# EarthyScience/EasyHybrid.jl

Measured on NVIDIA B200. Metric: training samples/sec (fwd+bwd+Adam), higher is better.
Workload: dtype f32

## Files before the change

### easyhybrid.jl_b200/csrc/eh_chunk.cuh

```cuda
#pragma once
#include "eh_pm.cuh"

namespace eh {

constexpr int MAXP = 12;
constexpr int EH_MAX_WORLD = 8;
constexpr int BS_C = 0, BS_N = MAXT, BS_SS = 2 * MAXT, BS_BN = 3 * MAXT, BS_AFF = 3 * MAXT + 2 * MAXP, BS_STRIDE = BS_AFF + 4 * MAXT;

enum : int { OPT_ADAM = 0, OPT_ADAMW = 1, OPT_RMSPROP = 2, OPT_DESCENT = 3 };
enum : int { UPD_FULL = 0, UPD_REDUCE_ONLY = 1, UPD_FROM_VECTOR = 2 };

struct OptState {
    float b1t, b2t;
    long long t;
    long long skipped;
};

struct PSlot {
    int role;
    int idx;
    float lo;
    float span;
    float fixedv;
};

template <int P_, int NH_, int H_, int NOUT_, int ACT_, bool SCALE_, class PM_, int SPL_ = 1>
struct StepCfg {
    static constexpr int P = P_, NH = NH_, H = H_, NOUT = NOUT_, ACT = ACT_;
    static constexpr bool SCALE = SCALE_;
    static constexpr int SPL = SPL_;
    static constexpr int CHUNKS = 32 * SPL_;
    static constexpr int RS = CHUNKS + 4;
    using PM = PM_;
    static constexpr int F = PM::NF, T = PM::NT, NPS = PM::NPS;
    static constexpr int LR = (NOUT_ * (H_ + 1) + PM_::NT + PM_::NPS <= 32) ? 1 : 0;
    static constexpr ShapeDims D{P_, NH_, H_, NOUT_, LR};
    static constexpr int NLAST = NOUT_ * (H_ + 1);
    static constexpr int R4 = rup4(P_ + PM::NF + PM::NT);
    static constexpr int NB = D.nblocks();
    static constexpr int NBI = (NB + 31) / 32;
    static constexpr int NBP = NB | 1;
    static constexpr int SCR_PAD = (NBP - NB) * 16;
    static constexpr int SCR = D.npart() + SCR_PAD;
    static constexpr int GS = 4 * RS + 4;
    static constexpr int AUXOFF = D.ngroups() * GS;
    static constexpr int STAGE_FLOATS = AUXOFF + (ACT_ == ACT_SWISH ? NH_ * H_ * RS : 0);
    static constexpr int NW = D.nweights();
    static constexpr int NPART = D.npart();
    static_assert(P_ <= MAXP && H_ % 4 == 0 && NOUT_ <= 4 && (SPL_ == 1 || SPL_ == 2), "shape limits");
};

constexpr int SS_SLOT = 0, SS_PMS = 16, SS_C = 48, SS_NV = 52, SS_BN = 56, SS_NV2 = 80, SS_SGD = 96, SS_AFF = 104, SS_FLOATS = 128;

template <int RS>
__device__ __forceinline__ constexpr int goff(int g0, int k) { return (g0 + (k >> 2)) * (4 * RS + 4) + (k & 3) * RS; }

__device__ __forceinline__ float comp(const float2* v, int k) { return (k & 1) ? v[k >> 1].y : v[k >> 1].x; }

template <int S>
__device__ __forceinline__ void stage_put(float* row, int lane, const float (&v)[S])
{
    if (S == 2) *reinterpret_cast<float2*>(row + 2 * lane) = f2(v[0], v[S - 1]);
    else row[lane] = v[0];
}
template <int S>
__device__ __forceinline__ void stage_get(const float* row, int lane, float (&v)[S])
{
    if (S == 2) {
        float2 t = *reinterpret_cast<const float2*>(row + 2 * lane);
        v[0] = t.x;
        v[S - 1] = t.y;
    } else {
        v[0] = row[lane];
    }
}

template <class C>
__device__ __forceinline__ float2 unit_act_fwd2(int l, int j2, float2 z, float2& aux)
// ... 42 lines not shown
        for (int k = 0; k < P; k++) {
            const float4* w4 = reinterpret_cast<const float4*>(sW + D.off_w1f() + k * H);
#pragma unroll
            for (int j = 0; j < HP; j += 2) {
                float4 w = w4[j >> 1];
                hp[j] = fma2s(f2(w.x, w.y), x[k], hp[j]);
                hp[j + 1] = fma2s(f2(w.z, w.w), x[k], hp[j + 1]);
            }
        }
    }
#pragma unroll
    for (int l = 1; l <= NH; l++) {
#pragma unroll
        for (int j = 0; j < HP; j++) {
            float2 aux = f2s(0.f);
            const float2 z = hp[j];
            hp[j] = unit_act_fwd2<C>(l, 2 * j, hp[j], aux);
            if (C::PM::DYNAMIC && pass) {
                const unsigned m = pass[l - 1] >> (2 * j);
                if (m & 1u) hp[j].x = z.x;
                if (m & 2u) hp[j].y = z.y;
            }
            if (STAGE && l + 1 <= D.nlt()) {
                stage[goff<RS>(D.gA(l + 1), 2 * j) + lane] = hp[j].x;
                stage[goff<RS>(D.gA(l + 1), 2 * j + 1) + lane] = hp[j].y;
            }
            if (STAGE) {
                if (C::ACT == ACT_SWISH) {
                    stage[C::AUXOFF + ((l - 1) * H + 2 * j) * RS + lane] = aux.x;
                    stage[C::AUXOFF + ((l - 1) * H + 2 * j + 1) * RS + lane] = aux.y;
                }
            }
        }
        if (l < NH) {
            float2 z[HP];
            const float4* b4 = reinterpret_cast<const float4*>(sW + D.off_b(l + 1));
#pragma unroll
            for (int j = 0; j < HP; j += 2) {
                float4 b = b4[j >> 1];
                z[j] = f2(b.x, b.y);
                z[j + 1] = f2(b.z, b.w);
            }
#pragma unroll
            for (int k = 0; k < H; k++) {
                const float4* w4 = reinterpret_cast<const float4*>(sW + D.off_wf(l + 1) + k * H);
                const float ak = comp(hp, k);
#pragma unroll
                for (int j = 0; j < HP; j += 2) {
// ... 47 lines not shown
    }
}

template <class C>
__device__ __forceinline__ void load_weights_and_scalars(const float* pblock, int nflat, const int* wsrc,
                                                         const float* bscal, int use_bn, float* sW, float* sS)
{
    for (int i = threadIdx.x; i < C::NW; i += blockDim.x) {
        int s = wsrc[i];
        sW[i] = s >= 0 ? __ldcg(pblock + s) : (s == -2 ? 1.f : 0.f);
    }
    if (threadIdx.x < MAXPS) sS[SS_SLOT + threadIdx.x] = __ldcg(pblock + nflat + threadIdx.x);
    if (threadIdx.x < MAXPS * PMS_PER_SLOT) sS[SS_PMS + threadIdx.x] = __ldcg(pblock + nflat + MAXPS + threadIdx.x);
    if (threadIdx.x < MAXT) sS[SS_C + threadIdx.x] = bscal ? bscal[BS_C + threadIdx.x] : 0.f;
    if (threadIdx.x < 2 * C::P)
        sS[SS_BN + threadIdx.x] = use_bn ? bscal[BS_BN + threadIdx.x] : ((threadIdx.x & 1) ? 1.f : 0.f);
    if (threadIdx.x < 3 * MAXT) sS[SS_AFF + threadIdx.x] = bscal ? bscal[BS_AFF + threadIdx.x] : 0.f;
}

template <class C>
__device__ __forceinline__ void init_stage_rows(float* stage, int lane)
{
    constexpr ShapeDims D = C::D;
    constexpr int RS = C::RS, S = C::SPL;
    float one[S], zero[S];
#pragma unroll
    for (int i = 0; i < S; i++) { one[i] = 1.f; zero[i] = 0.f; }
#pragma unroll
    for (int l = 1; l <= D.nlt(); l++) {
        const int din = D.din(l), ka = D.ka(l), gA = D.gA(l);
#pragma unroll
        for (int k = din; k < ka; k++) stage_put<S>(stage + goff<RS>(gA, k), lane, (k == din) ? one : zero);
    }
    if (!C::LR) {
#pragma unroll
        for (int o = C::NOUT; o < rup4(C::NOUT); o++) stage_put<S>(stage + goff<RS>(D.gD(C::NH + 1), o), lane, zero);
    }
}

template <class C>
__device__ __forceinline__ void tile_rows(int lane, int* rowD, int* rowA)
{
    constexpr ShapeDims D = C::D;
#pragma unroll
    for (int i = 0; i < C::NBI; i++) {
        int b = lane + 32 * i;
        rowD[i] = 0;
        rowA[i] = 0;
#pragma unroll
        for (int l = 1; l <= D.nlt(); l++) {
            const int b0 = D.blk0(l), nk = D.nk(l), nb = D.nj(l) * nk;
            if (b >= b0 && b < b0 + nb) {
                int jb = (b - b0) / nk, kb = (b - b0) % nk;
                rowD[i] = (D.gD(l) + jb) * C::GS;
                rowA[i] = (D.gA(l) + kb) * C::GS;
            }
        }
    }
}
// ... 35 lines not shown
        }
    }
};

template <class C>
__device__ __forceinline__ void chunk_sample_phase(const float (*rec)[C::R4], const bool* valid, const float* sW,
                                                   const float* sS, float* stage, int lane, const PSlot* slot,
                                                   const int* loss_kind, const PmCtx& cx, ChunkStats& st, LastAcc<C>& la)
{
    constexpr ShapeDims D = C::D;
    constexpr int P = C::P, NH = C::NH, H = C::H, NOUT = C::NOUT, T = C::T, F = C::F, NPS = C::NPS, HP = C::H / 2;
    constexpr int RS = C::RS, S = C::SPL;
    using PM = typename C::PM;

    float x[S][P];
#pragma unroll
    for (int k = 0; k < P; k++) {
        float v[S];
#pragma unroll
        for (int s = 0; s < S; s++) {
            x[s][k] = (rec[s][k] - sS[SS_BN + 2 * k]) * sS[SS_BN + 2 * k + 1];
            v[s] = x[s][k];
        }
        stage_put<S>(stage + goff<RS>(D.gA(1), k), lane, v);
    }

    float2 hp[S][HP];
    {
        const float4* b4 = reinterpret_cast<const float4*>(sW + D.off_b1());
#pragma unroll
        for (int j = 0; j < HP; j += 2) {
            float4 b = b4[j >> 1];
#pragma unroll
            for (int s = 0; s < S; s++) { hp[s][j] = f2(b.x, b.y); hp[s][j + 1] = f2(b.z, b.w); }
        }
#pragma unroll
        for (int k = 0; k < P; k++) {
            const float4* w4 = reinterpret_cast<const float4*>(sW + D.off_w1f() + k * H);
#pragma unroll
            for (int j = 0; j < HP; j += 2) {
                float4 w = w4[j >> 1];
#pragma unroll
                for (int s = 0; s < S; s++) {
                    hp[s][j] = fma2s(f2(w.x, w.y), x[s][k], hp[s][j]);
                    hp[s][j + 1] = fma2s(f2(w.z, w.w), x[s][k], hp[s][j + 1]);
                }
            }
        }
    }
#pragma unroll
    for (int l = 1; l <= NH; l++) {
#pragma unroll
        for (int j = 0; j < HP; j++) {
            float lo[S], hi[S], axl[S], axh[S];
#pragma unroll
            for (int s = 0; s < S; s++) {
                float2 aux = f2s(0.f);
                const float2 z = hp[s][j];
                hp[s][j] = unit_act_fwd2<C>(l, 2 * j, hp[s][j], aux);
                if (C::PM::DYNAMIC) {
                    const unsigned m = cx.pass[l - 1] >> (2 * j);
                    if (m & 1u) hp[s][j].x = z.x;
                    if (m & 2u) hp[s][j].y = z.y;
                }
                lo[s] = hp[s][j].x; hi[s] = hp[s][j].y; axl[s] = aux.x; axh[s] = aux.y;
            }
            if (l + 1 <= D.nlt()) {
                stage_put<S>(stage + goff<RS>(D.gA(l + 1), 2 * j), lane, lo);
                stage_put<S>(stage + goff<RS>(D.gA(l + 1), 2 * j + 1), lane, hi);
            }
            if (C::ACT == ACT_SWISH) {
                stage_put<S>(stage + C::AUXOFF + ((l - 1) * H + 2 * j) * RS, lane, axl);
                stage_put<S>(stage + C::AUXOFF + ((l - 1) * H + 2 * j + 1) * RS, lane, axh);
            }
        }
        if (l < NH) {
            float2 z[S][HP];
            const float4* b4 = reinterpret_cast<const float4*>(sW + D.off_b(l + 1));
#pragma unroll
            for (int j = 0; j < HP; j += 2) {
                float4 b = b4[j >> 1];
#pragma unroll
                for (int s = 0; s < S; s++) { z[s][j] = f2(b.x, b.y); z[s][j + 1] = f2(b.z, b.w); }
            }
#pragma unroll
            for (int k = 0; k < H; k++) {
                const float4* w4 = reinterpret_cast<const float4*>(sW + D.off_wf(l + 1) + k * H);
                float ak[S];
#pragma unroll
                for (int s = 0; s < S; s++) ak[s] = comp(hp[s], k);
#pragma unroll
                for (int j = 0; j < HP; j += 2) {
// ... 73 lines not shown
#pragma unroll
                for (int o = 0; o < NOUT; o++)
                    if (sl.idx == o) dz[s][o] += g;
            } else if (sl.role == ROLE_GLOBAL) {
                st.gphi[q] += gp[q];
            }
        }
    }
    if (C::LR) {
#pragma unroll
        for (int o = 0; o < NOUT; o++)
#pragma unroll
            for (int s = 0; s < S; s++) {
                la.b[o] += dz[s][o];
#pragma unroll
                for (int k = 0; k < HP; k++) la.w[o][k] = fma2s(hp[s][k], dz[s][o], la.w[o][k]);
            }
    } else {
#pragma unroll
        for (int o = 0; o < NOUT; o++) {
            float v[S];
#pragma unroll
            for (int s = 0; s < S; s++) v[s] = dz[s][o];
            stage_put<S>(stage + goff<RS>(D.gD(NH + 1), o), lane, v);
        }
    }

    float2 d[S][HP];
#pragma unroll
    for (int s = 0; s < S; s++)
#pragma unroll
        for (int k = 0; k < HP; k++) d[s][k] = f2s(0.f);
#pragma unroll
    for (int o = 0; o < NOUT; o++) {
        const float4* w4 = reinterpret_cast<const float4*>(sW + D.off_wo() + o * H);
#pragma unroll
        for (int k = 0; k < HP; k += 2) {
            float4 w = w4[k >> 1];
#pragma unroll
            for (int s = 0; s < S; s++) {
                d[s][k] = fma2s(f2(w.x, w.y), dz[s][o], d[s][k]);
                d[s][k + 1] = fma2s(f2(w.z, w.w), dz[s][o], d[s][k + 1]);
            }
        }
    }
#pragma unroll
    for (int l = NH; l >= 1; l--) {
#pragma unroll
        for (int k = 0; k < HP; k++) {
            float alo[S], ahi[S], xlo[S], xhi[S], dlo[S], dhi[S];
            if (l < NH) {
                stage_get<S>(stage + goff<RS>(D.gA(l + 1), 2 * k), lane, alo);
                stage_get<S>(stage + goff<RS>(D.gA(l + 1), 2 * k + 1), lane, ahi);
            }
            if (C::ACT == ACT_SWISH) {
                stage_get<S>(stage + C::AUXOFF + ((l - 1) * H + 2 * k) * RS, lane, xlo);
                stage_get<S>(stage + C::AUXOFF + ((l - 1) * H + 2 * k + 1) * RS, lane, xhi);
            }
#pragma unroll
            for (int s = 0; s < S; s++) {
                float2 al = (l < NH) ? f2(alo[s], ahi[s]) : hp[s][k];
                float2 aux = (C::ACT == ACT_SWISH) ? f2(xlo[s], xhi[s]) : f2s(0.f);
                float2 ga = unit_act_bwd2<C>(l, 2 * k, al, aux);
                if (C::PM::DYNAMIC) {
                    const unsigned m = cx.pass[l - 1] >> (2 * k);
                    if (m & 1u) ga.x = 1.f;
                    if (m & 2u) ga.y = 1.f;
                }
                d[s][k] = mul2(d[s][k], ga);
                dlo[s] = d[s][k].x;
                dhi[s] = d[s][k].y;
            }
            stage_put<S>(stage + goff<RS>(D.gD(l), 2 * k), lane, dlo);
            stage_put<S>(stage + goff<RS>(D.gD(l), 2 * k + 1), lane, dhi);
        }
        if (l > 1) {
            float2 dn[S][HP];
#pragma unroll
            for (int s = 0; s < S; s++)
#pragma unroll
                for (int k = 0; k < HP; k++) dn[s][k] = f2s(0.f);
#pragma unroll
            for (int j = 0; j < H; j++) {
                const float4* w4 = reinterpret_cast<const float4*>(sW + D.off_wb(l) + j * H);
                float dj[S];
#pragma unroll
                for (int s = 0; s < S; s++) dj[s] = comp(d[s], j);
#pragma unroll
                for (int k = 0; k < HP; k += 2) {
                    float4 w = w4[k >> 1];
#pragma unroll
                    for (int s = 0; s < S; s++) {
                        dn[s][k] = fma2s(f2(w.x, w.y), dj[s], dn[s][k]);
                        dn[s][k + 1] = fma2s(f2(w.z, w.w), dj[s], dn[s][k + 1]);
                    }
                }
            }
// ... 24 lines not shown
                float4 dv[4], av[4];
#pragma unroll
                for (int j = 0; j < 4; j++) dv[j] = *reinterpret_cast<const float4*>(pd + j * RS + c);
#pragma unroll
                for (int k = 0; k < 4; k++) av[k] = *reinterpret_cast<const float4*>(pa + k * RS + c);
#pragma unroll
                for (int j = 0; j < 4; j++)
#pragma unroll
                    for (int k = 0; k < 4; k++) {
                        acc[j * 4 + k] = fma2(f2(dv[j].x, dv[j].y), f2(av[k].x, av[k].y), acc[j * 4 + k]);
                        acc[j * 4 + k] = fma2(f2(dv[j].z, dv[j].w), f2(av[k].z, av[k].w), acc[j * 4 + k]);
                    }
            }
#pragma unroll
            for (int e = 0; e < 16; e++) wacc[e * C::NBP + b] = acc[e].x + acc[e].y;
        }
    }
}

template <class C>
__device__ __forceinline__ void chunk_dw_phase_mma(const float* stage, int lane, float* wacc, bool first)
{
    constexpr ShapeDims D = C::D;
    constexpr int RS = C::RS;
    static_assert(C::H % 16 == 0 && C::LR == 1 && C::SPL == 1, "tensor-pipe dW: hidden width multiple of 16, output layer in registers");
    constexpr int MT = C::H / 16;
    const int g = lane >> 2, t = lane & 3;
#pragma unroll
    for (int l = 1; l <= D.nlt(); l++) {
        const int ka = D.ka(l), nk = D.nk(l), b0 = D.blk0(l);
        const int NT = (ka + 7) / 8;
        float acc[MT][6][4];
#pragma unroll
        for (int mt = 0; mt < MT; mt++)
#pragma unroll
            for (int nt = 0; nt < 6; nt++)
#pragma unroll
                for (int q = 0; q < 4; q++) acc[mt][nt][q] = 0.f;
#pragma unroll
        for (int ks = 0; ks < C::CHUNKS / 8; ks++) {
            const int k0 = 8 * ks + t;
            unsigned bh[6][2], bl[6][2];
#pragma unroll
            for (int nt = 0; nt < 6; nt++) {
                if (nt < NT) {
                    const float* pb = stage + goff<RS>(D.gA(l), 8 * nt + g) + k0;
                    split_tf32(pb[0], bh[nt][0], bl[nt][0]);
                    split_tf32(pb[4], bh[nt][1], bl[nt][1]);
                }
            }
#pragma unroll
            for (int mt = 0; mt < MT; mt++) {
                const float* pa0 = stage + goff<RS>(D.gD(l), 16 * mt + g) + k0;
                const float* pa1 = stage + goff<RS>(D.gD(l), 16 * mt + g + 8) + k0;
                unsigned ah[4], al[4];
                split_tf32(pa0[0], ah[0], al[0]);
                split_tf32(pa1[0], ah[1], al[1]);
                split_tf32(pa0[4], ah[2], al[2]);
                split_tf32(pa1[4], ah[3], al[3]);
#pragma unroll
                for (int nt = 0; nt < 6; nt++)
                    if (nt < NT) mma_3xtf32(acc[mt][nt], ah, al, bh[nt], bl[nt]);
            }
        }
#pragma unroll
        for (int mt = 0; mt < MT; mt++)
#pragma unroll
            for (int nt = 0; nt < 6; nt++) {
                if (nt < NT) {
#pragma unroll
                    for (int q = 0; q < 4; q++) {
                        const int j = 16 * mt + g + ((q >> 1) ? 8 : 0), k = 8 * nt + 2 * t + (q & 1);
                        if (k < ka) {
                            const int cell = ((j & 3) * 4 + (k & 3)) * C::NBP + b0 + (j >> 2) * nk + (k >> 2);
                            wacc[cell] = first ? acc[mt][nt][q] : wacc[cell] + acc[mt][nt][q];
                        }
                    }
// ... 85 lines not shown
```

### easyhybrid.jl_b200/csrc/eh_engine_ffma.cuh

```cuda
#pragma once
#include "eh_chunk.cuh"

namespace eh {

template <class C>
struct EngFfma {
    using Cfg = C;
    static constexpr int ENGINE = C::SPL == 2 ? 2 : 0;
    static constexpr int STAGE_FLOATS = C::STAGE_FLOATS + rup4(C::SCR);
    static constexpr int NPART = C::NPART;
    static constexpr int OFF_STATS = C::D.npart_dw();
    static constexpr int CHUNK = C::CHUNKS;
    static constexpr int MAX_WARPS = C::SPL == 2 ? 10 : 16;
#ifdef EH_DW_FFMA
    static constexpr bool DW_MMA = false;
#else
    static constexpr bool DW_MMA = C::LR == 1 && C::H % 16 == 0 && C::SPL == 1 && C::D.ka(C::D.nlt()) <= 48;
#endif

    struct State {
        int nacc;
        ChunkStats st;
        LastAcc<C> la;
        int rowD[C::NBI], rowA[C::NBI];
        float4 r[C::SPL][C::R4 / 4];
        bool valid[C::SPL];
    };

    __device__ __forceinline__ static void init_warp(State& s, float* stage, int lane)
    {
        init_stage_rows<C>(stage, lane);
        tile_rows<C>(lane, s.rowD, s.rowA);
    }
    __device__ __forceinline__ static void after_reduce(State&, float*, int) {}
    __device__ __forceinline__ static void step_begin(State& s, const float* sW, int lane)
    {
        s.nacc = 0;
#pragma unroll
        for (int t = 0; t < MAXT; t++) s.st.loss[t] = 0.f;
#pragma unroll
        for (int t = 0; t < MAXPS; t++) s.st.gphi[t] = 0.f;
// ... 50 lines not shown
```

### easyhybrid.jl_b200/csrc/eh_engine_tc.cuh

```cuda
#pragma once
#include <cstdint>
#include "eh_engine_ffma.cuh"

namespace eh {

namespace tc {
constexpr int WPS = 256;
constexpr int ENG_WF_H = 0, ENG_WF_L = 4 * WPS, ENG_WB_H = 8 * WPS, ENG_WB_L = 12 * WPS, ENG_BAR = 16 * WPS, ENG_TMEM = ENG_BAR + 8 * 8,
              ENG_BYTES = ENG_TMEM + 16;
constexpr int COL_AH = 0, COL_AL = 16, COL_Z = 32, COLS_PER_GROUP = 64;

__device__ __forceinline__ uint32_t saddr(const void* p) { return (uint32_t)__cvta_generic_to_shared(p); }
__device__ __forceinline__ uint64_t desc(uint32_t sa, uint32_t lbo, uint32_t sbo)
{
    return (uint64_t)((sa & 0x3FFFF) >> 4) | ((uint64_t)((lbo >> 4) & 0x3FFF) << 16) | ((uint64_t)((sbo >> 4) & 0x3FFF) << 32) | ((uint64_t)1 << 46);
}
__host__ __device__ constexpr uint32_t idesc(int m, int n)
{
    return (1u << 4) | (2u << 7) | (2u << 10) | ((uint32_t)(n >> 3) << 17) | ((uint32_t)(m >> 4) << 24);
}
__device__ __forceinline__ void mma_ts(uint32_t d, uint32_t a, uint64_t b, uint32_t id, uint32_t acc)
{
    asm volatile(
        "{\n\t.reg .pred p;\n\tsetp.ne.b32 p, %4, 0;\n\t"
// ... 170 lines not shown
    __device__ __forceinline__ static void step_begin(State& s, const float*, int)
    {
        s.nacc = 0;
#pragma unroll
        for (int t = 0; t < MAXT; t++) s.st.loss[t] = 0.f;
#pragma unroll
        for (int t = 0; t < MAXPS; t++) s.st.gphi[t] = 0.f;
        s.la.zero();
    }
    __device__ __forceinline__ static void fetch(State& s, const FetchArgs& fa, int chunk, int lane)
    {
        const int smp = chunk * CHUNK + (((threadIdx.x >> 5) & 3) << 5) + lane;
        const bool v = chunk < fa.nchunks && smp < fa.B;
        s.valid = v;
#pragma unroll
        for (int q = 0; q < C::R4 / 4; q++) s.r[q] = v ? fetch_rec4<C::R4 / 4>(fa, smp, q) : make_float4(0.f, 0.f, 0.f, 0.f);
    }

    __device__ __forceinline__ static void chunk(State& s, const FetchArgs& fa, int next, const float* sW, const float* sS,
                                                 float* stage, int lane, const PSlot* slot, const int* loss_kind,
                                                 const PmCtx& cx, unsigned* err)
    {
        constexpr ShapeDims D = C::D;
        constexpr int P = C::P, H = C::H, NOUT = C::NOUT, T = C::T, NF = C::F, NPS = C::NPS, HP = C::H / 2, RS = C::RS;
        using PM = typename C::PM;
        const int warp = threadIdx.x >> 5, wq = warp & 3, g = warp >> 2;
        const bool leader = (wq == (g & 3)) && lane == 0;
        const uint32_t ph = s.tiles & 1u;
        const uint32_t tmg = s.tm & 0x0000ffffu;

        float rec[C::R4];
#pragma unroll
        for (int q = 0; q < C::R4 / 4; q++) {
            rec[4 * q] = s.r[q].x; rec[4 * q + 1] = s.r[q].y; rec[4 * q + 2] = s.r[q].z; rec[4 * q + 3] = s.r[q].w;
        }
        const bool valid = s.valid;
        fetch(s, fa, next, lane);

        float2 hp[HP];
        {
            float x[P];
#pragma unroll
            for (int k = 0; k < P; k++) {
                x[k] = (rec[k] - sS[SS_BN + 2 * k]) * sS[SS_BN + 2 * k + 1];
                stage[goff<RS>(D.gA(1), k) + lane] = x[k];
            }
            const float4* b4 = reinterpret_cast<const float4*>(sW + D.off_b1());
#pragma unroll
            for (int j = 0; j < HP; j += 2) {
                const float4 b = b4[j >> 1];
                hp[j] = f2(b.x, b.y);
                hp[j + 1] = f2(b.z, b.w);
            }
#pragma unroll
            for (int k = 0; k < P; k++) {
                const float4* w4 = reinterpret_cast<const float4*>(sW + D.off_w1f() + k * H);
#pragma unroll
                for (int j = 0; j < HP; j += 2) {
                    const float4 w = w4[j >> 1];
                    hp[j] = fma2s(f2(w.x, w.y), x[k], hp[j]);
                    hp[j + 1] = fma2s(f2(w.z, w.w), x[k], hp[j + 1]);
                }
            }
            float2 aux;
#pragma unroll
            for (int j = 0; j < HP; j++) {
                hp[j] = act_fwd2<C::ACT>(hp[j], aux);
                stage[goff<RS>(D.gA(2), 2 * j) + lane] = hp[j].x;
                stage[goff<RS>(D.gA(2), 2 * j + 1) + lane] = hp[j].y;
            }
        }
        tc::put_row(s.tm, hp);
        tc::fence_before();
        tc::group_sync(g);
        if (leader) {
            tc::fence_after();
            tc::issue(tmg, s.wf, s.wf + 4 * tc::WPS, s.bar);
        }
        {
            float z[16];
            tc::bar_wait(s.bar, ph, err);
            tc::fence_after();
            tc::ld16(s.tm + tc::COL_Z, z);
            const float4* b4 = reinterpret_cast<const float4*>(sW + D.off_b(2));
            float2 aux;
#pragma unroll
            for (int j = 0; j < HP; j += 2) {
                const float4 b = b4[j >> 1];
                hp[j] = act_fwd2<C::ACT>(add2(f2(z[2 * j], z[2 * j + 1]), f2(b.x, b.y)), aux);
                hp[j + 1] = act_fwd2<C::ACT>(add2(f2(z[2 * j + 2], z[2 * j + 3]), f2(b.z, b.w)), aux);
            }
        }
// ... 50 lines not shown
                    s.st.gphi[q] += gp[q];
                }
            }
        }
        float2 d[HP];
#pragma unroll
        for (int k = 0; k < HP; k++) d[k] = f2s(0.f);
#pragma unroll
        for (int o = 0; o < NOUT; o++) {
            s.la.b[o] += dz[o];
            const float4* w4 = reinterpret_cast<const float4*>(sW + D.off_wo() + o * H);
#pragma unroll
            for (int k = 0; k < HP; k += 2) {
                const float4 w = w4[k >> 1];
                s.la.w[o][k] = fma2s(hp[k], dz[o], s.la.w[o][k]);
                s.la.w[o][k + 1] = fma2s(hp[k + 1], dz[o], s.la.w[o][k + 1]);
                d[k] = fma2s(f2(w.x, w.y), dz[o], d[k]);
                d[k + 1] = fma2s(f2(w.z, w.w), dz[o], d[k + 1]);
            }
        }
#pragma unroll
        for (int k = 0; k < HP; k++) {
            d[k] = mul2(d[k], act_bwd2<C::ACT>(hp[k], f2s(0.f)));
            stage[goff<RS>(D.gD(2), 2 * k) + lane] = d[k].x;
            stage[goff<RS>(D.gD(2), 2 * k + 1) + lane] = d[k].y;
        }
        tc::put_row(s.tm, d);
        tc::fence_before();
        tc::group_sync(g);
        if (leader) {
            tc::fence_after();
            tc::issue(tmg, s.wb, s.wb + 4 * tc::WPS, s.bar + 8);
        }
        {
            float e[16];
            tc::bar_wait(s.bar + 8, ph, err);
            tc::fence_after();
            tc::ld16(s.tm + tc::COL_Z, e);
#pragma unroll
            for (int k = 0; k < HP; k++) {
                const float2 a1 = f2(stage[goff<RS>(D.gA(2), 2 * k) + lane], stage[goff<RS>(D.gA(2), 2 * k + 1) + lane]);
                const float2 d1 = mul2(f2(e[2 * k], e[2 * k + 1]), act_bwd2<C::ACT>(a1, f2s(0.f)));
                stage[goff<RS>(D.gD(1), 2 * k) + lane] = d1.x;
                stage[goff<RS>(D.gD(1), 2 * k + 1) + lane] = d1.y;
            }
        }
        tc::fence_before();
        __syncwarp();
        chunk_dw_phase_mma<C>(stage, lane, stage + C::STAGE_FLOATS, s.nacc == 0);
        s.nacc++;
        s.tiles++;
        __syncwarp();
    }

    __device__ __forceinline__ static void reduce_prepare(State& s, float* work, unsigned*)
    {
        cta_reduce_prepare<C>(s.nacc, s.st, s.la, work + C::STAGE_FLOATS, STAGE_FLOATS);
    }
    __device__ __forceinline__ static float reduce_sum_at(const float* work, int nw, int p)
    {
        return cta_reduce_sum_at<C>(work + C::STAGE_FLOATS, STAGE_FLOATS, nw, p);
    }
};

}
```

### easyhybrid.jl_b200/csrc/eh_epoch_kernel.cuh

```cuda
#pragma once
#include "eh_step_kernel.cuh"

namespace eh {

struct EpochArgs {
    const float4* rec;
    const int* idx;
    long long n;
    int B;
    long long first_step;
    int nsteps;
    int nb;
    float* pblock;
    int nflat, ntheta;
    float* m;
    float* v;
    OptState* ost;
    const int* wsrc;
    const int* pmap;
    const int* cells;
    const float* pspan;
    const int* slot_of_flat;
    const float* bscal;
    uint2* pbuf;
// ... 125 lines not shown
        : "=r"(ok) : "r"((unsigned)__cvta_generic_to_shared(bar)), "r"(parity) : "memory");
    return ok != 0;
}
__device__ __forceinline__ void mbar_wait(unsigned long long* bar, unsigned parity, unsigned* err, bool unbounded = false)
{
    unsigned spins = 0;
    while (!mbar_try_wait(bar, parity)) {
        if (!unbounded && ++spins > (1u << 22)) { *err = 1; break; }
    }
}
__device__ __forceinline__ void bulk_g2s(void* dst, const void* src, unsigned bytes, unsigned long long* bar)
{
    asm volatile("cp.async.bulk.shared::cluster.global.mbarrier::complete_tx::bytes [%0], [%1], %2, [%3];"
                 ::"r"((unsigned)__cvta_generic_to_shared(dst)), "l"(src), "r"(bytes), "r"((unsigned)__cvta_generic_to_shared(bar)) : "memory");
}

__device__ __forceinline__ void cta_chunk_range(int nchunks, int G, int bid, int& c0, int& cnt)
{
    const int base = nchunks / G, rem = nchunks - base * G;
    cnt = base + (bid < rem ? 1 : 0);
    c0 = bid * base + (bid < rem ? bid : rem);
}

__host__ __device__ constexpr int epoch_xbuf_floats(int npartp, int G) { return 4 * (npartp / 4 + G) + 8; }
__host__ __device__ constexpr int epoch_extra_floats(int npartp, int nflat, int tile_floats, int G)
{
    return npartp + 8 * rup4(nflat) + 2 * rup4(tile_floats) + 8 + epoch_xbuf_floats(npartp, G);
}

template <class E, class = void>
struct EngWpc { static constexpr int value = 1; };
template <class E>
struct EngWpc<E, decltype((void)E::WPC)> { static constexpr int value = E::WPC; };
template <class E>
constexpr int epoch_threads() { return EngWpc<E>::value > 1 ? (E::MAX_WARPS + 1) * 32 : ((E::MAX_WARPS + 1) * 32 > 512 ? 512 : (E::MAX_WARPS + 1) * 32); }

template <class E>
__global__ void __launch_bounds__(epoch_threads<E>(), 1) k_epoch(const EpochArgs a)
{
    constexpr int WPC = EngWpc<E>::value;
    using C = typename E::Cfg;
    extern __shared__ float4 smem4[];
    float* sW = reinterpret_cast<float*>(smem4);
    float* sS = sW + rup4(C::NW);
    const int lane = threadIdx.x & 31, warp = threadIdx.x >> 5, nwarps = blockDim.x >> 5;
    const int wcomp = a.wcomp;
    const bool service = warp == nwarps - 1;
    float* stage0 = sS + SS_FLOATS;
    float* stage = stage0 + (service ? 0 : warp) * E::STAGE_FLOATS;
    float* red = stage0 + a.work_floats;
    float* s_th = red + a.npartp;
    float* s_m = s_th + rup4(a.nflat);
    float* s_v = s_m + rup4(a.nflat);
    int* t_pmap = reinterpret_cast<int*>(s_v + rup4(a.nflat));
    int* t_cell0 = t_pmap + rup4(a.nflat);
    int* t_cell1 = t_cell0 + rup4(a.nflat);
    int* t_slot = t_cell1 + rup4(a.nflat);
    float* t_span = reinterpret_cast<float*>(t_slot + rup4(a.nflat));
    float4* tile0 = reinterpret_cast<float4*>(t_span + rup4(a.nflat));
    unsigned long long* mbar = reinterpret_cast<unsigned long long*>(reinterpret_cast<float*>(tile0) + 2 * rup4(a.tile_floats));
    unsigned* phi_flag = reinterpret_cast<unsigned*>(mbar + 2);
    float2* xbuf = reinterpret_cast<float2*>(phi_flag + 4);
    const int G = gridDim.x, bid = blockIdx.x;
    unsigned char* eng = reinterpret_cast<unsigned char*>(smem4) + a.eng_off;
    const int unit = warp / WPC, nunits = wcomp / WPC;
    if constexpr (WPC > 1) E::cta_init(eng);
    const bool tiles = a.tile_floats > 0;
    constexpr int R44 = C::R4 / 4;

    for (int p = threadIdx.x; p < a.nflat; p += blockDim.x) {
        s_th[p] = a.pblock[p];
        s_m[p] = a.m[p];
        s_v[p] = a.v[p];
        t_pmap[p] = a.pmap[p];
        t_cell0[p] = a.cells[2 * p];
        t_cell1[p] = a.cells[2 * p + 1];
        t_slot[p] = a.slot_of_flat[p];
        t_span[p] = a.pspan[p];
        if (p >= a.ntheta && p - a.ntheta < MAXPS) {
            const float sg0 = 1.f / (1.f + expf(-a.pblock[p]));
            sS[SS_SGD + p - a.ntheta] = a.pspan[p] * sg0 * (1.f - sg0);
        }
    }
    float b1t = a.ost->b1t, b2t = a.ost->b2t;
    long long tdone = 0, tskip = 0;
    if (threadIdx.x == 0) {
        mbar_init(&mbar[0], 1);
        mbar_init(&mbar[1], 1);
        *phi_flag = a.tag_base;
        phi_flag[1] = 0u;
        asm volatile("fence.mbarrier_init.release.cluster;" ::: "memory");
    }

    typename E::State st;
    if constexpr (WPC == 1) {
        if (!service) E::init_warp(st, stage, lane);
    }
    load_weights_and_scalars<C>(a.pblock, a.nflat, a.wsrc, nullptr, 0, sW, sS);
    __syncthreads();
    if constexpr (WPC > 1) {
        E::load_w2(eng, sW);
        asm volatile("fence.proxy.async.shared::cta;" ::: "memory");
        if (!service) E::init_warp(st, stage, lane, eng);
    }

    PmCtx cx;
    cx.pms = sS + SS_PMS;
    cx.c = a.pmc;
// ... 145 lines not shown
        if constexpr (WPC == 1) {
            if (E::SCRATCH_ALIASES_STAGE) {
                __syncthreads();
                if (!service) E::reduce_prepare(st, stage0);
            }
        }
        __syncthreads();
        EH_STAMP(2)
        if (service && have_next) store_bs(pre, s + 1);

        for (int p0 = 0; p0 < a.npartp; p0 += blockDim.x) {
            const int p = p0 + threadIdx.x;
            const float v0 = p < E::NPART ? E::reduce_sum_at(stage0, wcomp, p) : 0.f;
            const float v1 = __shfl_down_sync(0xffffffffu, v0, 1);
            if (p < a.npartp && !(p & 1)) {
                const int k = p >> 1;
                if (G == 1) *reinterpret_cast<float2*>(red + p) = make_float2(v0, v1);
                else st_cg_v4(part + ((size_t)(k >> 1) * Gp + bid) * 4 + (k & 1) * 2, __float_as_uint(v0), tag, __float_as_uint(v1), tag);
            }
        }
        EH_STAMP(3)
        const float rb1 = 1.f / (1.f - b1t), rb2 = 1.f / (1.f - b2t);
        if (G > 1) {
            const int nitems = 2 * G * nown;
            for (int i = threadIdx.x; i < nitems; i += blockDim.x) {
                const int row = i / (2 * G), rem = i - row * 2 * G, half = rem & 1, peer = rem >> 1;
                const uint4 v = poll_pair_cg(part + (size_t)(bid + row * G) * Gp * 4 + rem * 2, tag, a.err);
                xbuf[(row * 2 + half) * G + peer] = make_float2(__uint_as_float(v.x), __uint_as_float(v.z));
            }
            __syncthreads();
            {
                const unsigned dtag = a.step_base + (unsigned)s + 1u;
                const int dpar = (int)((a.step_base + (unsigned)s) & 1u);
                for (int pr = nwarps - 1 - warp; pr < 2 * nown; pr += nwarps) {
                    EH_STAMP_SVC(24)
                    const float2* src = xbuf + (size_t)pr * G;
                    float acc0 = 0.f, acc1 = 0.f;
                    for (int c = lane; c < G; c += 32) { const float2 v = src[c]; acc0 += v.x; acc1 += v.y; }
                    for (int o = 16; o > 0; o >>= 1) {
                        acc0 += __shfl_xor_sync(0xffffffffu, acc0, o);
                        acc1 += __shfl_xor_sync(0xffffffffu, acc1, o);
                    }
                    const int ge = (bid + (pr >> 1) * G) * 4 + (pr & 1) * 2;
                    if (a.world > 1) {
                        float v0 = 0.f, v1 = 0.f;
                        if (lane < a.world) {
                            st_volatile_v4(a.inbox_peer[lane] + ((size_t)dpar * a.world + a.rank) * a.npartp + ge, __float_as_uint(acc0), dtag,
                                           __float_as_uint(acc1), dtag);
                            const uint2* in = a.inbox_peer[a.rank] + ((size_t)dpar * a.world + lane) * a.npartp + ge;
                            const uint4 v = poll_pair(in, ld_volatile_v4(in), dtag, a.err);
                            v0 = __uint_as_float(v.x);
                            v1 = __uint_as_float(v.z);
                        }
                        acc0 = 0.f; acc1 = 0.f;
                        for (int r = 0; r < a.world; r++) {
                            acc0 += __shfl_sync(0xffffffffu, v0, r);
                            acc1 += __shfl_sync(0xffffffffu, v1, r);
                        }
                    }
                    if (lane < EH_TOT_REPL) st_cg_v4(tot + (size_t)lane * a.npartp + ge, __float_as_uint(acc0), tag, __float_as_uint(acc1), tag);
                    EH_STAMP_SVC(25)
                }
            }
            for (int k = threadIdx.x; k < a.npartp / 2; k += blockDim.x) {
                const uint4 v = poll_pair_cg(mytot + 2 * k, tag, a.err);
                *reinterpret_cast<float2*>(red + 2 * k) = make_float2(__uint_as_float(v.x), __uint_as_float(v.z));
            }
        }
        __syncthreads();
        if (service) bar_arrive_id(1, blockDim.x);
        EH_STAMP(4)

        float ntot = 0.f, post = 1.f;
        for (int t = 0; t < a.T; t++) {
            const float nv = sS[SS_NV2 + par * MAXT + t];
            ntot += nv;
            if (a.loss_kind[t] == LOSS_RMSE) post = 1.f / (2.f * sqrtf(red[E::OFF_STATS + t] / nv));
        }
        const bool skip = ntot == 0.f;
        if (bid == 0 && service) {
            if (lane < MAXT) a.stats_out[(size_t)s * MAXT + lane] = red[E::OFF_STATS + lane];
            if (stream && lane == 0) {
                float L = 0.f;
                for (int t = 0; t < a.T; t++) {
                    const float nv = sS[SS_NV2 + par * MAXT + t], acc = red[E::OFF_STATS + t];
                    L += a.loss_kind[t] == LOSS_RMSE ? sqrtf(acc / nv) : acc / nv;
                }
                if (a.agg_mean) L /= (float)a.T;
                a.loss_stream[s] = skip ? __int_as_float(0x7fc00000) : L;
                *reinterpret_cast<volatile unsigned*>(a.done) = a.ready_base + (unsigned)s + 1u;
            }
        }
        const int pbeg = service ? a.ntheta + lane : threadIdx.x;
        const int pend = service ? a.nflat : a.ntheta;
        const int pstep = service ? 32 : ncomp_threads;
        if (!skip) {
            for (int p = pbeg; p < pend; p += pstep) {
                float g = red[t_pmap[p]] * post;
                float th = s_th[p];
                const bool phi_cached = p >= a.ntheta && p - a.ntheta < MAXPS;
                if (phi_cached) {
                    g *= sS[SS_SGD + p - a.ntheta];
                } else if (p >= a.ntheta) {
                    float sg = 1.f / (1.f + expf(-th));
                    g *= t_span[p] * sg * (1.f - sg);
                }
                float dx;
                if (a.opt_kind == OPT_ADAM || a.opt_kind == OPT_ADAMW) {
                    float mt = a.beta1 * s_m[p] + (1.f - a.beta1) * g;
                    float vt = a.beta2 * s_v[p] + (1.f - a.beta2) * g * g;
                    s_m[p] = mt;
                    s_v[p] = vt;
                    dx = mt * rb1 / (sqrtf(vt * rb2) + a.eps) * a.eta;
                    if (a.opt_kind == OPT_ADAMW) dx += (a.adamw_coupled ? a.eta * a.lambda : a.lambda) * th;
                } else if (a.opt_kind == OPT_RMSPROP) {
                    float qv = a.beta2 * s_v[p] + (1.f - a.beta2) * g * g;
                    s_v[p] = qv;
                    dx = g * a.eta / (sqrtf(qv) + a.eps);
                } else {
                    dx = a.eta * g;
                }
                th -= dx;
                s_th[p] = th;
                const int c0 = t_cell0[p], c1 = t_cell1[p];
                if (c0 >= 0) sW[c0] = th;
                if (c1 >= 0) sW[c1] = th;
                if constexpr (WPC > 1) {
                    if (c0 >= 0) E::patch_cell(eng, c0, th);
                    if (c1 >= 0) E::patch_cell(eng, c1, th);
                }
                if (p >= a.ntheta) {
                    const float sgn = 1.f / (1.f + expf(-th));
                    if (phi_cached) sS[SS_SGD + p - a.ntheta] = t_span[p] * sgn * (1.f - sgn);
                    const int sl = t_slot[p];
                    if (sl >= 0) {
                        const PSlot ps = a.slot[sl];
                        float val = ps.lo + ps.span * sgn;
                        float o4[4];
                        pm_prep_slot_fast(a.pm_id, sl, val, o4);
                        sS[SS_SLOT + sl] = val;
                        for (int i = 0; i < 4; i++) sS[SS_PMS + sl * PMS_PER_SLOT + i] = o4[i];
                    }
                }
            }
            b1t *= a.beta1;
            b2t *= a.beta2;
            tdone++;
        } else {
            tskip++;
        }
        EH_STAMP(5)
        if (service) {
            __syncwarp();
            __threadfence_block();
            if (lane == 0) asm volatile("st.volatile.shared.u32 [%0], %1;" ::"r"((unsigned)__cvta_generic_to_shared(phi_flag)), "r"(tag) : "memory");
            EH_STAMP_SVC(27)
            if (stream && !have_next && s + 1 < a.nsteps) {
                if (wait_slot(s + 1, bnext)) {
                    store_bs(load_bs(bnext), s + 1);
                    __syncwarp();
                    if (lane == 0) issue_tile(bnext, par ^ 1);
                } else {
                    if (lane == 0) {
                        *stop_flag = 1u;
                        __threadfence_block();
                        mbar_arrive(&mbar[par ^ 1]);
                    }
                    __syncwarp();
                }
            }
        }
        if (!service) {
            if constexpr (WPC > 1) asm volatile("fence.proxy.async.shared::cta;" ::: "memory");
            bar_sync_id(1, blockDim.x);
            E::after_reduce(st, stage, lane);
        }
        bcur = bnext;
        EH_STAMP(6)
    }
#undef EH_STAMP
#undef EH_STAMP_SVC

    __syncthreads();
    if constexpr (WPC > 1) E::cta_exit(eng);
    if (bid == 0) {
        for (int p = threadIdx.x; p < a.nflat; p += blockDim.x) {
            a.pblock[p] = s_th[p];
            a.m[p] = s_m[p];
            a.v[p] = s_v[p];
        }
        if (threadIdx.x < MAXPS) a.pblock[a.nflat + threadIdx.x] = sS[SS_SLOT + threadIdx.x];
        if (threadIdx.x < MAXPS * PMS_PER_SLOT) a.pblock[a.nflat + MAXPS + threadIdx.x] = sS[SS_PMS + threadIdx.x];
        if (threadIdx.x == 0) {
            a.ost->b1t = b1t;
            a.ost->b2t = b2t;
            a.ost->t += tdone;
            a.ost->skipped += tskip;
        }
    }
}

}
```

Measured before the change: 5.629 billion.

## Stream cross-block gradient reduction directly from global and pack optimizer state

```diff
diff --git a/easyhybrid.jl_b200/csrc/eh_chunk.cuh b/easyhybrid.jl_b200/csrc/eh_chunk.cuh
--- a/easyhybrid.jl_b200/csrc/eh_chunk.cuh
+++ b/easyhybrid.jl_b200/csrc/eh_chunk.cuh
@@ -42,7 +42,12 @@
     static constexpr int NBP = NB | 1;
     static constexpr int SCR_PAD = (NBP - NB) * 16;
     static constexpr int SCR = D.npart() + SCR_PAD;
-    static constexpr int GS = 4 * RS + 4;
+#ifdef EH_DW_FFMA
+    static constexpr bool DW_MMA = false;
+#else
+    static constexpr bool DW_MMA = LR == 1 && H_ % 16 == 0 && SPL_ == 1 && D.ka(D.nlt()) <= 48;
+#endif
+    static constexpr int GS = 4 * RS + (DW_MMA ? 0 : 4);
     static constexpr int AUXOFF = D.ngroups() * GS;
     static constexpr int STAGE_FLOATS = AUXOFF + (ACT_ == ACT_SWISH ? NH_ * H_ * RS : 0);
     static constexpr int NW = D.nweights();
@@ -52,8 +57,8 @@
 
 constexpr int SS_SLOT = 0, SS_PMS = 16, SS_C = 48, SS_NV = 52, SS_BN = 56, SS_NV2 = 80, SS_SGD = 96, SS_AFF = 104, SS_FLOATS = 128;
 
-template <int RS>
-__device__ __forceinline__ constexpr int goff(int g0, int k) { return (g0 + (k >> 2)) * (4 * RS + 4) + (k & 3) * RS; }
+template <class C>
+__device__ __forceinline__ constexpr int goff(int g0, int k) { return (g0 + (k >> 2)) * C::GS + (k & 3) * C::RS; }
 
 __device__ __forceinline__ float comp(const float2* v, int k) { return (k & 1) ? v[k >> 1].y : v[k >> 1].x; }
 
@@ -142,8 +147,8 @@
                 if (m & 2u) hp[j].y = z.y;
             }
             if (STAGE && l + 1 <= D.nlt()) {
-                stage[goff<RS>(D.gA(l + 1), 2 * j) + lane] = hp[j].x;
-                stage[goff<RS>(D.gA(l + 1), 2 * j + 1) + lane] = hp[j].y;
+                stage[goff<C>(D.gA(l + 1), 2 * j) + lane] = hp[j].x;
+                stage[goff<C>(D.gA(l + 1), 2 * j + 1) + lane] = hp[j].y;
             }
             if (STAGE) {
                 if (C::ACT == ACT_SWISH) {
@@ -237,7 +242,7 @@
 __device__ __forceinline__ void init_stage_rows(float* stage, int lane)
 {
     constexpr ShapeDims D = C::D;
-    constexpr int RS = C::RS, S = C::SPL;
+    constexpr int S = C::SPL;
     float one[S], zero[S];
 #pragma unroll
     for (int i = 0; i < S; i++) { one[i] = 1.f; zero[i] = 0.f; }
@@ -245,11 +250,11 @@
     for (int l = 1; l <= D.nlt(); l++) {
         const int din = D.din(l), ka = D.ka(l), gA = D.gA(l);
 #pragma unroll
-        for (int k = din; k < ka; k++) stage_put<S>(stage + goff<RS>(gA, k), lane, (k == din) ? one : zero);
+        for (int k = din; k < ka; k++) stage_put<S>(stage + goff<C>(gA, k), lane, (k == din) ? one : zero);
     }
     if (!C::LR) {
 #pragma unroll
-        for (int o = C::NOUT; o < rup4(C::NOUT); o++) stage_put<S>(stage + goff<RS>(D.gD(C::NH + 1), o), lane, zero);
+        for (int o = C::NOUT; o < rup4(C::NOUT); o++) stage_put<S>(stage + goff<C>(D.gD(C::NH + 1), o), lane, zero);
     }
 }
 
@@ -331,7 +336,7 @@
             x[s][k] = (rec[s][k] - sS[SS_BN + 2 * k]) * sS[SS_BN + 2 * k + 1];
             v[s] = x[s][k];
         }
-        stage_put<S>(stage + goff<RS>(D.gA(1), k), lane, v);
+        stage_put<S>(stage + goff<C>(D.gA(1), k), lane, v);
     }
 
     float2 hp[S][HP];
@@ -375,8 +380,8 @@
                 lo[s] = hp[s][j].x; hi[s] = hp[s][j].y; axl[s] = aux.x; axh[s] = aux.y;
             }
             if (l + 1 <= D.nlt()) {
-                stage_put<S>(stage + goff<RS>(D.gA(l + 1), 2 * j), lane, lo);
-                stage_put<S>(stage + goff<RS>(D.gA(l + 1), 2 * j + 1), lane, hi);
+                stage_put<S>(stage + goff<C>(D.gA(l + 1), 2 * j), lane, lo);
+                stage_put<S>(stage + goff<C>(D.gA(l + 1), 2 * j + 1), lane, hi);
             }
             if (C::ACT == ACT_SWISH) {
                 stage_put<S>(stage + C::AUXOFF + ((l - 1) * H + 2 * j) * RS, lane, axl);
@@ -496,7 +501,7 @@
             float v[S];
 #pragma unroll
             for (int s = 0; s < S; s++) v[s] = dz[s][o];
-            stage_put<S>(stage + goff<RS>(D.gD(NH + 1), o), lane, v);
+            stage_put<S>(stage + goff<C>(D.gD(NH + 1), o), lane, v);
         }
     }
 
@@ -524,8 +529,8 @@
         for (int k = 0; k < HP; k++) {
             float alo[S], ahi[S], xlo[S], xhi[S], dlo[S], dhi[S];
             if (l < NH) {
-                stage_get<S>(stage + goff<RS>(D.gA(l + 1), 2 * k), lane, alo);
-                stage_get<S>(stage + goff<RS>(D.gA(l + 1), 2 * k + 1), lane, ahi);
+                stage_get<S>(stage + goff<C>(D.gA(l + 1), 2 * k), lane, alo);
+                stage_get<S>(stage + goff<C>(D.gA(l + 1), 2 * k + 1), lane, ahi);
             }
             if (C::ACT == ACT_SWISH) {
                 stage_get<S>(stage + C::AUXOFF + ((l - 1) * H + 2 * k) * RS, lane, xlo);
@@ -545,8 +550,8 @@
                 dlo[s] = d[s][k].x;
                 dhi[s] = d[s][k].y;
             }
-            stage_put<S>(stage + goff<RS>(D.gD(l), 2 * k), lane, dlo);
-            stage_put<S>(stage + goff<RS>(D.gD(l), 2 * k + 1), lane, dhi);
+            stage_put<S>(stage + goff<C>(D.gD(l), 2 * k), lane, dlo);
+            stage_put<S>(stage + goff<C>(D.gD(l), 2 * k + 1), lane, dhi);
         }
         if (l > 1) {
             float2 dn[S][HP];
@@ -617,7 +622,6 @@
 __device__ __forceinline__ void chunk_dw_phase_mma(const float* stage, int lane, float* wacc, bool first)
 {
     constexpr ShapeDims D = C::D;
-    constexpr int RS = C::RS;
     static_assert(C::H % 16 == 0 && C::LR == 1 && C::SPL == 1, "tensor-pipe dW: hidden width multiple of 16, output layer in registers");
     constexpr int MT = C::H / 16;
     const int g = lane >> 2, t = lane & 3;
@@ -639,15 +643,15 @@
 #pragma unroll
             for (int nt = 0; nt < 6; nt++) {
                 if (nt < NT) {
-                    const float* pb = stage + goff<RS>(D.gA(l), 8 * nt + g) + k0;
+                    const float* pb = stage + goff<C>(D.gA(l), 8 * nt + g) + k0;
                     split_tf32(pb[0], bh[nt][0], bl[nt][0]);
                     split_tf32(pb[4], bh[nt][1], bl[nt][1]);
                 }
             }
 #pragma unroll
             for (int mt = 0; mt < MT; mt++) {
-                const float* pa0 = stage + goff<RS>(D.gD(l), 16 * mt + g) + k0;
-                const float* pa1 = stage + goff<RS>(D.gD(l), 16 * mt + g + 8) + k0;
+                const float* pa0 = stage + goff<C>(D.gD(l), 16 * mt + g) + k0;
+                const float* pa1 = stage + goff<C>(D.gD(l), 16 * mt + g + 8) + k0;
                 unsigned ah[4], al[4];
                 split_tf32(pa0[0], ah[0], al[0]);
                 split_tf32(pa1[0], ah[1], al[1]);
diff --git a/easyhybrid.jl_b200/csrc/eh_engine_ffma.cuh b/easyhybrid.jl_b200/csrc/eh_engine_ffma.cuh
--- a/easyhybrid.jl_b200/csrc/eh_engine_ffma.cuh
+++ b/easyhybrid.jl_b200/csrc/eh_engine_ffma.cuh
@@ -12,11 +12,7 @@
     static constexpr int OFF_STATS = C::D.npart_dw();
     static constexpr int CHUNK = C::CHUNKS;
     static constexpr int MAX_WARPS = C::SPL == 2 ? 10 : 16;
-#ifdef EH_DW_FFMA
-    static constexpr bool DW_MMA = false;
-#else
-    static constexpr bool DW_MMA = C::LR == 1 && C::H % 16 == 0 && C::SPL == 1 && C::D.ka(C::D.nlt()) <= 48;
-#endif
+    static constexpr bool DW_MMA = C::DW_MMA;
 
     struct State {
         int nacc;
diff --git a/easyhybrid.jl_b200/csrc/eh_engine_tc.cuh b/easyhybrid.jl_b200/csrc/eh_engine_tc.cuh
--- a/easyhybrid.jl_b200/csrc/eh_engine_tc.cuh
+++ b/easyhybrid.jl_b200/csrc/eh_engine_tc.cuh
@@ -216,7 +216,7 @@
                                                  const PmCtx& cx, unsigned* err)
     {
         constexpr ShapeDims D = C::D;
-        constexpr int P = C::P, H = C::H, NOUT = C::NOUT, T = C::T, NF = C::F, NPS = C::NPS, HP = C::H / 2, RS = C::RS;
+        constexpr int P = C::P, H = C::H, NOUT = C::NOUT, T = C::T, NF = C::F, NPS = C::NPS, HP = C::H / 2;
         using PM = typename C::PM;
         const int warp = threadIdx.x >> 5, wq = warp & 3, g = warp >> 2;
         const bool leader = (wq == (g & 3)) && lane == 0;
@@ -237,7 +237,7 @@
 #pragma unroll
             for (int k = 0; k < P; k++) {
                 x[k] = (rec[k] - sS[SS_BN + 2 * k]) * sS[SS_BN + 2 * k + 1];
-                stage[goff<RS>(D.gA(1), k) + lane] = x[k];
+                stage[goff<C>(D.gA(1), k) + lane] = x[k];
             }
             const float4* b4 = reinterpret_cast<const float4*>(sW + D.off_b1());
 #pragma unroll
@@ -260,8 +260,8 @@
 #pragma unroll
             for (int j = 0; j < HP; j++) {
                 hp[j] = act_fwd2<C::ACT>(hp[j], aux);
-                stage[goff<RS>(D.gA(2), 2 * j) + lane] = hp[j].x;
-                stage[goff<RS>(D.gA(2), 2 * j + 1) + lane] = hp[j].y;
+                stage[goff<C>(D.gA(2), 2 * j) + lane] = hp[j].x;
+                stage[goff<C>(D.gA(2), 2 * j + 1) + lane] = hp[j].y;
             }
         }
         tc::put_row(s.tm, hp);
@@ -358,8 +358,8 @@
 #pragma unroll
         for (int k = 0; k < HP; k++) {
             d[k] = mul2(d[k], act_bwd2<C::ACT>(hp[k], f2s(0.f)));
-            stage[goff<RS>(D.gD(2), 2 * k) + lane] = d[k].x;
-            stage[goff<RS>(D.gD(2), 2 * k + 1) + lane] = d[k].y;
+            stage[goff<C>(D.gD(2), 2 * k) + lane] = d[k].x;
+            stage[goff<C>(D.gD(2), 2 * k + 1) + lane] = d[k].y;
         }
         tc::put_row(s.tm, d);
         tc::fence_before();
@@ -375,10 +375,10 @@
             tc::ld16(s.tm + tc::COL_Z, e);
 #pragma unroll
             for (int k = 0; k < HP; k++) {
-                const float2 a1 = f2(stage[goff<RS>(D.gA(2), 2 * k) + lane], stage[goff<RS>(D.gA(2), 2 * k + 1) + lane]);
+                const float2 a1 = f2(stage[goff<C>(D.gA(2), 2 * k) + lane], stage[goff<C>(D.gA(2), 2 * k + 1) + lane]);
                 const float2 d1 = mul2(f2(e[2 * k], e[2 * k + 1]), act_bwd2<C::ACT>(a1, f2s(0.f)));
-                stage[goff<RS>(D.gD(1), 2 * k) + lane] = d1.x;
-                stage[goff<RS>(D.gD(1), 2 * k + 1) + lane] = d1.y;
+                stage[goff<C>(D.gD(1), 2 * k) + lane] = d1.x;
+                stage[goff<C>(D.gD(1), 2 * k + 1) + lane] = d1.y;
             }
         }
         tc::fence_before();
diff --git a/easyhybrid.jl_b200/csrc/eh_epoch_kernel.cuh b/easyhybrid.jl_b200/csrc/eh_epoch_kernel.cuh
--- a/easyhybrid.jl_b200/csrc/eh_epoch_kernel.cuh
+++ b/easyhybrid.jl_b200/csrc/eh_epoch_kernel.cuh
@@ -171,10 +171,9 @@
     c0 = bid * base + (bid < rem ? bid : rem);
 }
 
-__host__ __device__ constexpr int epoch_xbuf_floats(int npartp, int G) { return 4 * (npartp / 4 + G) + 8; }
 __host__ __device__ constexpr int epoch_extra_floats(int npartp, int nflat, int tile_floats, int G)
 {
-    return npartp + 8 * rup4(nflat) + 2 * rup4(tile_floats) + 8 + epoch_xbuf_floats(npartp, G);
+    return npartp + 8 * rup4(nflat) + 2 * rup4(tile_floats) + 8 + (4 * (npartp / 4 + G) + 8);
 }
 
 template <class E, class = void>
@@ -198,18 +197,13 @@
     float* stage0 = sS + SS_FLOATS;
     float* stage = stage0 + (service ? 0 : warp) * E::STAGE_FLOATS;
     float* red = stage0 + a.work_floats;
-    float* s_th = red + a.npartp;
-    float* s_m = s_th + rup4(a.nflat);
-    float* s_v = s_m + rup4(a.nflat);
-    int* t_pmap = reinterpret_cast<int*>(s_v + rup4(a.nflat));
-    int* t_cell0 = t_pmap + rup4(a.nflat);
-    int* t_cell1 = t_cell0 + rup4(a.nflat);
-    int* t_slot = t_cell1 + rup4(a.nflat);
+    float4* s_ent = reinterpret_cast<float4*>(red + a.npartp);
+    int2* t_cells = reinterpret_cast<int2*>(s_ent + a.nflat);
+    int* t_slot = reinterpret_cast<int*>(t_cells + rup4(a.nflat));
     float* t_span = reinterpret_cast<float*>(t_slot + rup4(a.nflat));
     float4* tile0 = reinterpret_cast<float4*>(t_span + rup4(a.nflat));
     unsigned long long* mbar = reinterpret_cast<unsigned long long*>(reinterpret_cast<float*>(tile0) + 2 * rup4(a.tile_floats));
     unsigned* phi_flag = reinterpret_cast<unsigned*>(mbar + 2);
-    float2* xbuf = reinterpret_cast<float2*>(phi_flag + 4);
     const int G = gridDim.x, bid = blockIdx.x;
     unsigned char* eng = reinterpret_cast<unsigned char*>(smem4) + a.eng_off;
     const int unit = warp / WPC, nunits = wcomp / WPC;
@@ -218,12 +212,8 @@
     constexpr int R44 = C::R4 / 4;
 
     for (int p = threadIdx.x; p < a.nflat; p += blockDim.x) {
-        s_th[p] = a.pblock[p];
-        s_m[p] = a.m[p];
-        s_v[p] = a.v[p];
-        t_pmap[p] = a.pmap[p];
-        t_cell0[p] = a.cells[2 * p];
-        t_cell1[p] = a.cells[2 * p + 1];
+        s_ent[p] = make_float4(a.pblock[p], a.m[p], a.v[p], __int_as_float(a.pmap[p]));
+        t_cells[p] = make_int2(a.cells[2 * p], a.cells[2 * p + 1]);
         t_slot[p] = a.slot_of_flat[p];
         t_span[p] = a.pspan[p];
         if (p >= a.ntheta && p - a.ntheta < MAXPS) {
@@ -232,7 +222,7 @@
         }
     }
     float b1t = a.ost->b1t, b2t = a.ost->b2t;
-    long long tdone = 0, tskip = 0;
+    int tdone = 0;
     if (threadIdx.x == 0) {
         mbar_init(&mbar[0], 1);
         mbar_init(&mbar[1], 1);
@@ -424,21 +414,37 @@
         EH_STAMP(3)
         const float rb1 = 1.f / (1.f - b1t), rb2 = 1.f / (1.f - b2t);
         if (G > 1) {
-            const int nitems = 2 * G * nown;
-            for (int i = threadIdx.x; i < nitems; i += blockDim.x) {
-                const int row = i / (2 * G), rem = i - row * 2 * G, half = rem & 1, peer = rem >> 1;
-                const uint4 v = poll_pair_cg(part + (size_t)(bid + row * G) * Gp * 4 + rem * 2, tag, a.err);
-                xbuf[(row * 2 + half) * G + peer] = make_float2(__uint_as_float(v.x), __uint_as_float(v.z));
-            }
-            __syncthreads();
             {
                 const unsigned dtag = a.step_base + (unsigned)s + 1u;
                 const int dpar = (int)((a.step_base + (unsigned)s) & 1u);
                 for (int pr = nwarps - 1 - warp; pr < 2 * nown; pr += nwarps) {
                     EH_STAMP_SVC(24)
-                    const float2* src = xbuf + (size_t)pr * G;
+                    const uint2* src = part + (size_t)(bid + (pr >> 1) * G) * Gp * 4 + (pr & 1) * 2;
                     float acc0 = 0.f, acc1 = 0.f;
-                    for (int c = lane; c < G; c += 32) { const float2 v = src[c]; acc0 += v.x; acc1 += v.y; }
+                    constexpr int NPL = 5;
+                    for (int c0 = lane; c0 < G; c0 += 32 * NPL) {
+                        uint4 v[NPL];
+#pragma unroll
+                        for (int i = 0; i < NPL; i++)
+                            v[i] = c0 + 32 * i < G ? ld_cg_v4(src + (size_t)(c0 + 32 * i) * 4) : make_uint4(0u, tag, 0u, tag);
+                        for (unsigned spins = 0;;) {
+                            bool stale = false;
+#pragma unroll
+                            for (int i = 0; i < NPL; i++) stale |= v[i].y != tag || v[i].w != tag;
+                            if (!stale) break;
+                            if (++spins > EH_SPIN_LIMIT) { *a.err = 1; break; }
+#pragma unroll
+                            for (int i = 0; i < NPL; i++)
+                                if (v[i].y != tag || v[i].w != tag) v[i] = ld_cg_v4(src + (size_t)(c0 + 32 * i) * 4);
+                        }
+#pragma unroll
+                        for (int i = 0; i < NPL; i++) {
+                            if (c0 + 32 * i < G) {
+                                acc0 += __uint_as_float(v[i].x);
+                                acc1 += __uint_as_float(v[i].z);
+                            }
+                        }
+                    }
                     for (int o = 16; o > 0; o >>= 1) {
                         acc0 += __shfl_xor_sync(0xffffffffu, acc0, o);
                         acc1 += __shfl_xor_sync(0xffffffffu, acc1, o);
@@ -464,12 +470,14 @@
                     EH_STAMP_SVC(25)
                 }
             }
-            for (int k = threadIdx.x; k < a.npartp / 2; k += blockDim.x) {
-                const uint4 v = poll_pair_cg(mytot + 2 * k, tag, a.err);
-                *reinterpret_cast<float2*>(red + 2 * k) = make_float2(__uint_as_float(v.x), __uint_as_float(v.z));
-            }
-        }
-        __syncthreads();
+        } else {
+            __syncthreads();
+        }
+        auto total_at = [&](int e) {
+            if (G == 1) return red[e];
+            const uint4 v = poll_pair_cg(mytot + (e & ~1), tag, a.err);
+            return __uint_as_float((e & 1) ? v.z : v.x);
+        };
         if (service) bar_arrive_id(1, blockDim.x);
         EH_STAMP(4)
 
@@ -477,29 +485,35 @@
         for (int t = 0; t < a.T; t++) {
             const float nv = sS[SS_NV2 + par * MAXT + t];
             ntot += nv;
-            if (a.loss_kind[t] == LOSS_RMSE) post = 1.f / (2.f * sqrtf(red[E::OFF_STATS + t] / nv));
+            if (a.loss_kind[t] == LOSS_RMSE) post = 1.f / (2.f * sqrtf(total_at(E::OFF_STATS + t) / nv));
         }
         const bool skip = ntot == 0.f;
         if (bid == 0 && service) {
-            if (lane < MAXT) a.stats_out[(size_t)s * MAXT + lane] = red[E::OFF_STATS + lane];
-            if (stream && lane == 0) {
+            const float stat = lane < MAXT ? total_at(E::OFF_STATS + lane) : 0.f;
+            if (lane < MAXT) a.stats_out[(size_t)s * MAXT + lane] = stat;
+            if (stream) {
                 float L = 0.f;
                 for (int t = 0; t < a.T; t++) {
-                    const float nv = sS[SS_NV2 + par * MAXT + t], acc = red[E::OFF_STATS + t];
+                    const float nv = sS[SS_NV2 + par * MAXT + t], acc = __shfl_sync(0xffffffffu, stat, t);
                     L += a.loss_kind[t] == LOSS_RMSE ? sqrtf(acc / nv) : acc / nv;
                 }
                 if (a.agg_mean) L /= (float)a.T;
-                a.loss_stream[s] = skip ? __int_as_float(0x7fc00000) : L;
-                *reinterpret_cast<volatile unsigned*>(a.done) = a.ready_base + (unsigned)s + 1u;
+                if (lane == 0) {
+                    a.loss_stream[s] = skip ? __int_as_float(0x7fc00000) : L;
+                    *reinterpret_cast<volatile unsigned*>(a.done) = a.ready_base + (unsigned)s + 1u;
+                }
             }
         }
         const int pbeg = service ? a.ntheta + lane : threadIdx.x;
         const int pend = service ? a.nflat : a.ntheta;
         const int pstep = service ? 32 : ncomp_threads;
-        if (!skip) {
-            for (int p = pbeg; p < pend; p += pstep) {
-                float g = red[t_pmap[p]] * post;
-                float th = s_th[p];
+        for (int p = pbeg; p < pend; p += pstep) {
+            float4 ent = s_ent[p];
+            const float gsum = total_at(__float_as_int(ent.w));
+            if (p == 0) EH_STAMP(7)
+            if (!skip) {
+                float g = gsum * post;
+                float th = ent.x;
                 const bool phi_cached = p >= a.ntheta && p - a.ntheta < MAXPS;
                 if (phi_cached) {
                     g *= sS[SS_SGD + p - a.ntheta];
@@ -509,22 +523,24 @@
                 }
                 float dx;
                 if (a.opt_kind == OPT_ADAM || a.opt_kind == OPT_ADAMW) {
-                    float mt = a.beta1 * s_m[p] + (1.f - a.beta1) * g;
-                    float vt = a.beta2 * s_v[p] + (1.f - a.beta2) * g * g;
-                    s_m[p] = mt;
-                    s_v[p] = vt;
+                    float mt = a.beta1 * ent.y + (1.f - a.beta1) * g;
+                    float vt = a.beta2 * ent.z + (1.f - a.beta2) * g * g;
+                    ent.y = mt;
+                    ent.z = vt;
                     dx = mt * rb1 / (sqrtf(vt * rb2) + a.eps) * a.eta;
                     if (a.opt_kind == OPT_ADAMW) dx += (a.adamw_coupled ? a.eta * a.lambda : a.lambda) * th;
                 } else if (a.opt_kind == OPT_RMSPROP) {
-                    float qv = a.beta2 * s_v[p] + (1.f - a.beta2) * g * g;
-                    s_v[p] = qv;
+                    float qv = a.beta2 * ent.z + (1.f - a.beta2) * g * g;
+                    ent.z = qv;
                     dx = g * a.eta / (sqrtf(qv) + a.eps);
                 } else {
                     dx = a.eta * g;
                 }
                 th -= dx;
-                s_th[p] = th;
-                const int c0 = t_cell0[p], c1 = t_cell1[p];
+                ent.x = th;
+                s_ent[p] = ent;
+                const int2 cl = t_cells[p];
+                const int c0 = cl.x, c1 = cl.y;
                 if (c0 >= 0) sW[c0] = th;
                 if (c1 >= 0) sW[c1] = th;
                 if constexpr (WPC > 1) {
@@ -545,11 +561,11 @@
                     }
                 }
             }
+        }
+        if (!skip) {
             b1t *= a.beta1;
             b2t *= a.beta2;
             tdone++;
-        } else {
-            tskip++;
         }
         EH_STAMP(5)
         if (service) {
@@ -587,9 +603,10 @@
     if constexpr (WPC > 1) E::cta_exit(eng);
     if (bid == 0) {
         for (int p = threadIdx.x; p < a.nflat; p += blockDim.x) {
-            a.pblock[p] = s_th[p];
-            a.m[p] = s_m[p];
-            a.v[p] = s_v[p];
+            const float4 e = s_ent[p];
+            a.pblock[p] = e.x;
+            a.m[p] = e.y;
+            a.v[p] = e.z;
         }
         if (threadIdx.x < MAXPS) a.pblock[a.nflat + threadIdx.x] = sS[SS_SLOT + threadIdx.x];
         if (threadIdx.x < MAXPS * PMS_PER_SLOT) a.pblock[a.nflat + MAXPS + threadIdx.x] = sS[SS_PMS + threadIdx.x];
@@ -597,9 +614,9 @@
             a.ost->b1t = b1t;
             a.ost->b2t = b2t;
             a.ost->t += tdone;
-            a.ost->skipped += tskip;
-        }
-    }
-}
-
-}
+            a.ost->skipped += s_end - tdone;
+        }
+    }
+}
+
+}
```

Result: no change. 5.660 billion (median of 6 runs) (+0.5%).
